# oscka/rag-llm-k8s

Measured on AMD Instinct MI355X. Metric: end-to-end RAG query p50 latency + gen tokens/sec, Llama-3.1-8B top-k=4, higher is better.
Workload: dtype bf16; 1 GPU; model=Llama-3.1-8B-Instruct, embedder=all-MiniLM-L6-v2, index=FlatL2 10000 vectors (HBM-resident; 10000 embedded chunks), retrieve_k=4, context_k=4, global_batch=32, seq_len=5192, parallelism=dp1

## Files before the change

### csrc/kernels/attention.hip

```cpp
#include "common.h"
#include "kv_fp8.h"
#include <type_traits>
using namespace ragk;

namespace {

constexpr int KT = 64;
constexpr int MAX_BT = 2048;
constexpr float RESCALE_LOG2 = 8.f;

__device__ __forceinline__ float max_xor32(float v) {
  const auto r = __builtin_amdgcn_permlane32_swap(__float_as_uint(v), __float_as_uint(v), false, false);
  return fmaxf(__uint_as_float(r[0]), __uint_as_float(r[1]));
}
__device__ __forceinline__ float max_xor16(float v) {
  const auto r = __builtin_amdgcn_permlane16_swap(__float_as_uint(v), __float_as_uint(v), false, false);
  return fmaxf(__uint_as_float(r[0]), __uint_as_float(r[1]));
}

template <int D>
struct Cfg {
  static constexpr int NC = D / 8;
  static constexpr int ROWB = D * 2;
  static constexpr int TILEB = KT * D * 2;
  static constexpr int PIECES = TILEB / 1024;
  static constexpr int RPP = 1024 / ROWB;
  static constexpr int KS = D / 32;
  static constexpr int DT = D / 16;
  static constexpr int GR = D / 16;
  static constexpr int RB = 8 / GR;
};

template <int D>
__device__ __forceinline__ int kswz(int row) {
  constexpr int NC = Cfg<D>::NC;
  return (row / (16 / NC)) & (NC - 1);
}
template <int D>
__device__ __forceinline__ int vswz(int row) {
  return 2 * ((row / Cfg<D>::RB) & (Cfg<D>::GR - 1));
}

__device__ __forceinline__ bf16x4 tr_read(const char* p) {
  return __builtin_amdgcn_ds_read_tr16_b64_v4i16((__attribute__((address_space(3))) bf16x4*)(p));
}

template <int D, bool IS_V, bool NT = false, int NW = 0, typename RowSrc>
__device__ __forceinline__ void stage_kv(char* lds_tile, int wid, int nwaves, int lane, RowSrc row_src) {
  constexpr int NC = Cfg<D>::NC, PIECES = Cfg<D>::PIECES, RPP = Cfg<D>::RPP;
  constexpr int PPW = NW > 0 ? PIECES / NW : PIECES;
#pragma unroll
  for (int i = 0; i < PPW; ++i) {
    const int p = NW > 0 ? wid + NW * i : wid + nwaves * i;
    if (NW == 0 && p >= PIECES) break;
    const int row = p * RPP + lane / NC;
    const int ph = lane % NC;
    const int c = ph ^ (IS_V ? vswz<D>(row) : kswz<D>(row));
    if constexpr (NT)
      __builtin_amdgcn_global_load_lds((const __attribute__((address_space(1))) void*)(row_src(row) + c * 8),
                                       (__attribute__((address_space(3))) void*)(lds_tile + p * 1024), 16, 0, 2);
    else
      glds16(row_src(row) + c * 8, lds_tile + p * 1024);
  }
}

template <int D>
__device__ __forceinline__ bf16x8 load_vt(const char* sV, int dt, int ks, int lane) {
  const int h = lane >> 4, i = lane & 15;
  const int chunk = 2 * dt + ((i >> 1) & 1);
  const int r0 = 32 * ks + 4 * h + (i >> 2);
  const int r1 = r0 + 16;
  const bf16x4 a = tr_read(sV + r0 * Cfg<D>::ROWB + 16 * (chunk ^ vswz<D>(r0)) + 8 * (i & 1));
  const bf16x4 b = tr_read(sV + r1 * Cfg<D>::ROWB + 16 * (chunk ^ vswz<D>(r1)) + 8 * (i & 1));
  return (bf16x8){a[0], a[1], a[2], a[3], b[0], b[1], b[2], b[3]};
}

template <int D>
__device__ __forceinline__ bf16x8 load_k(const char* sK, int t, int s, int lane) {
  const int R = 16 * t + (lane & 15);
  const int c = 4 * s + (lane >> 4);
  return *reinterpret_cast<const bf16x8*>(sK + R * Cfg<D>::ROWB + 16 * (c ^ kswz<D>(R)));
}

__device__ __forceinline__ bf16x8 pack_p(const f32x4& a, const f32x4& b) {
  return (bf16x8){f2bf_s(a[0]), f2bf_s(a[1]), f2bf_s(a[2]), f2bf_s(a[3]),
                  f2bf_s(b[0]), f2bf_s(b[1]), f2bf_s(b[2]), f2bf_s(b[3])};
}

constexpr int F8_D = 128;
constexpr int F8_TILEB = KT * F8_D;

__device__ __forceinline__ int f8_qoff(int s, int fh) { return 64 * (s >> 1) + 16 * fh + 8 * (s & 1); }

template <bool NT>
__device__ __forceinline__ u32x4 f8_ld16(const unsigned char* p) {
  if constexpr (NT) return __builtin_nontemporal_load(reinterpret_cast<const u32x4*>(p));
  else return *reinterpret_cast<const u32x4*>(p);
}

__device__ __forceinline__ void f8_v_to_lds(char* sV, int ci, const u32x4 raw) {
  const int row = ci >> 3, c = ci & 7;
  char* p = sV + row * Cfg<F8_D>::ROWB + 16 * ((2 * c) ^ vswz<F8_D>(row));
  *reinterpret_cast<bf16x8*>(p) = kv8_to_bf16(raw[0], raw[1]);
  *reinterpret_cast<bf16x8*>(p + 16) = kv8_to_bf16(raw[2], raw[3]);
}

__device__ __forceinline__ void f8_load_k(const char* sK, int t, int j, int lane, bf16x8& k0, bf16x8& k1) {
  const u32x4 raw = __builtin_bit_cast(u32x4, load_k<64>(sK, t, j, lane));
  k0 = kv8_to_bf16(raw[0], raw[1]);
  k1 = kv8_to_bf16(raw[2], raw[3]);
}

struct PrefillArgs {
  const bf16_t* q;  int q_stride;
  const bf16_t* k;  const bf16_t* v;
  int kv_stride;
  const int* block_tables; int bt_stride;
  const int* cu_q;
  const int* cu_kv;
  const int* kv_lens;
  const int* tiles;
  bf16_t* out; int out_stride;
  int Hq, Hkv;
  float scale_log2;
  unsigned kv_bytes;
  int n_hg;
  const float* ks; const float* vs;
};

__device__ inline void prefill_block(const PrefillArgs& a, int& tile, int& hg) {
  if (a.n_hg > 0) {
    tile = (int)blockIdx.x / a.n_hg;
    hg = (int)blockIdx.x - tile * a.n_hg;
  } else {
    tile = blockIdx.x;
    hg = blockIdx.y;
  }
}

template <int D, int GB, bool CAUSAL, bool PAGED, int NWV = 4, bool F8 = false>
__global__ __launch_bounds__(NWV * 64, 8 / NWV) void attn_prefill_kernel(PrefillArgs a) {
  static_assert(!F8 || (PAGED && D == F8_D), "fp8 cache: paged, D = 128");
  using C = Cfg<D>;
  constexpr int NTH = NWV * 64;
  constexpr int QT = 32 * (NWV / GB);
// ... 540 lines not shown
      fast(P3{}, t + 2, S1, S0);
      fast(P0{}, t + 3, S0, S1);
    }
    if (t < t_end) {
      fast(P1{}, t, S1, S0);
      ++t;
    }
    if (t < t_end) {
      fast(P2{}, t, S0, S1);
      ++t;
    }
    if (t < t_end) {
      fast(P3{}, t, S1, S0);
      ++t;
    }
    if (t & 1) {
#pragma unroll
      for (int kb = 0; kb < 2; ++kb) S0[kb] = S1[kb];
    }
  }
  if (t + 2 < n_kt) stage(t + 2, true);
  wait_vmcnt0();
  barrier();
  if (t >= 1) pv_simple(t - 1);
  for (; t < n_kt; ++t) {
    const int k0 = t * KT;
    const bool need_mask = (k0 + KT - 1 > ctx0 + pbase) || (k0 + KT > kv_len);
    const float alpha = need_mask ? softmax(std::true_type{}, k0, S0) : softmax(std::false_type{}, k0, S0);
    rescale(alpha);
    pv_simple(t);
    if (t + 1 < n_kt) qk_simple(t + 1, S0);
  }

  const auto lr = __builtin_amdgcn_permlane32_swap(__float_as_uint(l_i), __float_as_uint(l_i), false, false);
  const float l = __uint_as_float(lr[0]) + __uint_as_float(lr[1]);
  const float inv = l > 0.f ? 1.f / l : 0.f;
  __syncthreads();
  char* so = smem + wid_u * 8192;
#pragma unroll
  for (int db = 0; db < 4; ++db)
#pragma unroll
    for (int b = 0; b < 4; ++b) {
      const int e = 4 * b;
      const int d = 32 * db + 8 * b + 4 * h;
      const int c = (d >> 3) ^ (l32 & 15);
      *reinterpret_cast<uint2*>(so + l32 * 256 + 16 * c + 8 * ((d >> 2) & 1)) =
          make_uint2(pk2bf(o[db][e] * inv, o[db][e + 1] * inv), pk2bf(o[db][e + 2] * inv, o[db][e + 3] * inv));
    }
  asm volatile("s_waitcnt lgkmcnt(0)" ::: "memory");
#pragma unroll
  for (int i = 0; i < 8; ++i) {
    const int r = 4 * i + (lane >> 4), c = lane & 15;
    const u32x4 v = *reinterpret_cast<const u32x4*>(so + r * 256 + 16 * (c ^ (r & 15)));
    if (pbase + r < q_len)
      *reinterpret_cast<u32x4*>(a.out + (size_t)(q_off + pbase + r) * a.out_stride + hq * D + 8 * c) = v;
  }
}

struct DecodeArgs {
  const bf16_t* q; int q_stride;
  const bf16_t* kc; const bf16_t* vc;
  const int* block_tables; int bt_stride;
  const int* kv_lens;
  float* part_o;
  float* part_ml;
  bf16_t* out; int out_stride;
  int Hq, Hkv, part_tiles, max_parts;
  float scale_log2;
  const float* qkv_p; long long p_slab; int ldp, S;
  const int* positions; const int* slots;
  const float* cos_t; const float* sin_t;
  const float* ks; const float* vs;
};

__device__ __forceinline__ int decode_part_tiles(int n_kt, const DecodeArgs& a) {
  return max(a.part_tiles, (n_kt + a.max_parts - 1) / a.max_parts);
}

template <int D, int G, int NW = 4, bool KL = false, bool F8 = false>
constexpr int decode_lds_bytes() {
  return F8 ? NW * (Cfg<D>::TILEB + (KL ? F8_TILEB : 0)) + G * D * 2 : NW * Cfg<D>::TILEB * (KL ? 2 : 1) + G * D * 2;
}

template <int D, int G, bool NT = false, int NW = 4, int DG = 0, bool KL = false, bool F8 = false>
__device__ __forceinline__ void attn_decode_block(const DecodeArgs& a, int part, int kvh, int b, char* smem) {
  constexpr int NTH = NW * 64;
  using C = Cfg<D>;
  static_assert(G <= 16, "at most 16 query heads per KV head");
  static_assert(!F8 || (D == F8_D && DG == 0), "fp8 cache: D = 128");
  const int lane = threadIdx.x & 63, wid = threadIdx.x >> 6;
  const int wid_u = __builtin_amdgcn_readfirstlane(wid);
  const int kv_len = a.kv_lens[b];
  const int n_kt = (kv_len + KT - 1) / KT;
  const int pt = decode_part_tiles(n_kt, a);
  const int kt0 = part * pt;
  if (kt0 >= n_kt) return;
  const int kt1 = min(kt0 + pt, n_kt);
  const int nparts = (n_kt + pt - 1) / pt;
  const int fr = lane & 15, fh = lane >> 4;
  const int* bt = a.block_tables + (size_t)b * a.bt_stride;

  bf16x8 qf[C::KS];
  char* sV = smem + wid * C::TILEB;
  char* sK = F8 ? smem + NW * C::TILEB + wid * F8_TILEB : smem + (NW + wid) * C::TILEB;
  const bool pre = !F8 && a.qkv_p != nullptr && kt0 + wid_u < kt1 && kt0 + wid_u != n_kt - 1;
  bf16x8 kf0[4][C::KS];
  if (pre) {
    const size_t base = ((size_t)bt[kt0 + wid_u] * a.Hkv + kvh) * KT * D;
    const bf16_t* kb = a.kc + base;
    const bf16_t* vb = a.vc + base;
    if constexpr (KL) stage_kv<D, false, NT, 1>(sK, 0, 1, lane, [&](int r) { return kb + (size_t)r * D; });
    stage_kv<D, true, NT, 1>(sV, 0, 1, lane, [&](int r) { return vb + (size_t)r * D; });
#pragma unroll
    for (int t = 0; t < 4; ++t)
#pragma unroll
      for (int s = 0; s < C::KS; ++s)
        if constexpr (!KL)
          kf0[t][s] = NT ? __builtin_nontemporal_load(reinterpret_cast<const bf16x8*>(kb + (size_t)(16 * t + fr) * D +
                                                                                     32 * s + 8 * fh))
                         : *reinterpret_cast<const bf16x8*>(kb + (size_t)(16 * t + fr) * D + 32 * s + 8 * fh);
  }
  if (a.qkv_p != nullptr) {
    bf16_t* s_q = reinterpret_cast<bf16_t*>(smem + decode_lds_bytes<D, G, NW, KL, F8>() - G * D * 2);
    constexpr int NV = D / 16;
    const int pos = a.positions[b];
    const float* prow = a.qkv_p + (size_t)b * a.ldp;
    const float* ct = a.cos_t + (size_t)pos * (D / 2);
    const float* st = a.sin_t + (size_t)pos * (D / 2);
    const int tid = threadIdx.x;
    const bool append = kt1 == n_kt;
    constexpr int KV0 = (G * NV + 63) / 64 * 64;
    if (tid < G * NV) {
      const int g = tid / NV, v = tid % NV;
      const float* ph = prow + (size_t)(kvh * G + g) * D + 8 * v;
      float x1[8], x2[8], o1[8], o2[8];
      sum_partials8x2(ph, ph + D / 2, a.S, (size_t)a.p_slab, x1, x2);
      rope8(x1, x2, ct + 8 * v, st + 8 * v, o1, o2);
      *reinterpret_cast<u32x4*>(s_q + g * D + 8 * v) = pack8(o1);
      *reinterpret_cast<u32x4*>(s_q + g * D + D / 2 + 8 * v) = pack8(o2);
    } else if (append && tid >= KV0 && tid < KV0 + 2 * NV) {
      const int isv = tid - KV0 >= NV, v = (tid - KV0) % NV;
      const int slot = a.slots[b];
      const size_t kvo = (((size_t)(slot / KT) * a.Hkv + kvh) * KT + (slot % KT)) * D;
      const float* ph = prow + (size_t)(a.Hq + (isv ? a.Hkv : 0) + kvh) * D + 8 * v;
      float x1[8], x2[8];
      sum_partials8x2(ph, ph + D / 2, a.S, (size_t)a.p_slab, x1, x2);
      bf16_t* dst = (isv ? const_cast<bf16_t*>(a.vc) : const_cast<bf16_t*>(a.kc)) + kvo;
      if constexpr (F8) {
        float r1[8], r2[8];
        if (isv) {
#pragma unroll
          for (int e = 0; e < 8; ++e) { r1[e] = x1[e]; r2[e] = x2[e]; }
        } else {
          rope8(x1, x2, ct + 8 * v, st + 8 * v, r1, r2);
        }
        unsigned char* base8 = reinterpret_cast<unsigned char*>(const_cast<bf16_t*>(isv ? a.vc : a.kc));
        kv8_store_row128(r1, r2, v, base8 + kvo, const_cast<float*>(isv ? a.vs : a.ks) + kvo / D);
      } else if (isv) {
        *reinterpret_cast<u32x4*>(dst + 8 * v) = pack8(x1);
        *reinterpret_cast<u32x4*>(dst + D / 2 + 8 * v) = pack8(x2);
      } else {
        float o1[8], o2[8];
        rope8(x1, x2, ct + 8 * v, st + 8 * v, o1, o2);
        *reinterpret_cast<u32x4*>(dst + 8 * v) = pack8(o1);
        *reinterpret_cast<u32x4*>(dst + D / 2 + 8 * v) = pack8(o2);
      }
    }
    __syncthreads();
#pragma unroll
    for (int s = 0; s < C::KS; ++s)
      qf[s] = fr < G ? *reinterpret_cast<const bf16x8*>(s_q + fr * D + (F8 ? f8_qoff(s, fh) : 32 * s + 8 * fh))
                     : (bf16x8){0, 0, 0, 0, 0, 0, 0, 0};
  } else {
    const int g = fr < G ? fr : 0;
    const bf16_t* qp = a.q + (size_t)b * a.q_stride + (kvh * G + g) * D + 8 * fh;
#pragma unroll
    for (int s = 0; s < C::KS; ++s) {
      const bf16x8 v = *reinterpret_cast<const bf16x8*>(F8 ? qp - 8 * fh + f8_qoff(s, fh) : qp + 32 * s);
      qf[s] = fr < G ? v : (bf16x8){0, 0, 0, 0, 0, 0, 0, 0};
    }
  }
  f32x4 o[C::DT];
#pragma unroll
  for (int dt = 0; dt < C::DT; ++dt) o[dt] = (f32x4){0.f, 0.f, 0.f, 0.f};
  float m_i = -INFINITY, l_i = 0.f;
  unsigned dsink = 0;

  for (int kt = kt0 + wid_u; kt < kt1; kt += NW) {
    bf16x8 kf[4][C::KS];
    u32x4 f8_v[F8 ? 8 : 1];
    f32x4 ksc[4], vsc[4];
    if constexpr (F8) {
      const size_t blk = (size_t)bt[kt] * a.Hkv + kvh;
      const unsigned char* kb = reinterpret_cast<const unsigned char*>(a.kc) + blk * F8_TILEB;
      const unsigned char* vb = reinterpret_cast<const unsigned char*>(a.vc) + blk * F8_TILEB;
      asm volatile("s_waitcnt lgkmcnt(0)" ::: "memory");
      if constexpr (KL)
        stage_kv<64, false, NT, 1>(sK, 0, 1, lane,
                                   [&](int r) { return reinterpret_cast<const bf16_t*>(kb + (size_t)r * F8_D); });
      u32x4 kraw[4][2];
      if constexpr (!KL) {
#pragma unroll
        for (int t = 0; t < 4; ++t)
#pragma unroll
          for (int j = 0; j < 2; ++j) kraw[t][j] = f8_ld16<NT>(kb + (16 * t + fr) * F8_D + 16 * (4 * j + fh));
      }
#pragma unroll
      for (int t = 0; t < 4; ++t) {
        ksc[t] = *reinterpret_cast<const f32x4*>(a.ks + blk * KT + 16 * t + 4 * fh);
        vsc[t] = *reinterpret_cast<const f32x4*>(a.vs + blk * KT + 16 * t + 4 * fh);
      }
#pragma unroll
      for (int i = 0; i < 8; ++i) f8_v[i] = f8_ld16<NT>(vb + 16 * (64 * i + lane));
      if constexpr (KL) {
        __builtin_amdgcn_s_waitcnt((0x7 << 4) | (0xF << 8));
#pragma unroll
        for (int t = 0; t < 4; ++t)
#pragma unroll
          for (int j = 0; j < 2; ++j) f8_load_k(sK, t, j, lane, kf[t][2 * j], kf[t][2 * j + 1]);
      } else {
#pragma unroll
        for (int t = 0; t < 4; ++t)
#pragma unroll
          for (int j = 0; j < 2; ++j) {
            kf[t][2 * j] = kv8_to_bf16(kraw[t][j][0], kraw[t][j][1]);
            kf[t][2 * j + 1] = kv8_to_bf16(kraw[t][j][2], kraw[t][j][3]);
          }
      }
    } else if constexpr (KL) {
      if (!(pre && kt == kt0 + wid_u)) {
        const size_t base = ((size_t)bt[kt] * a.Hkv + kvh) * KT * D;
        const bf16_t* kb = a.kc + base;
        const bf16_t* vb = a.vc + base;
        asm volatile("s_waitcnt lgkmcnt(0)" ::: "memory");
        stage_kv<D, false, NT, 1>(sK, 0, 1, lane, [&](int r) { return kb + (size_t)r * D; });
        stage_kv<D, true, NT, 1>(sV, 0, 1, lane, [&](int r) { return vb + (size_t)r * D; });
      }
      static_assert(Cfg<D>::PIECES < 64, "vmcnt range");
      __builtin_amdgcn_s_waitcnt((Cfg<D>::PIECES & 15) | (((Cfg<D>::PIECES >> 4) & 3) << 14) | (0x7 << 4) | (0xF << 8));
#pragma unroll
      for (int t = 0; t < 4; ++t)
#pragma unroll
        for (int s = 0; s < C::KS; ++s) kf[t][s] = load_k<D>(sK, t, s, lane);
    } else if (pre && kt == kt0 + wid_u) {
#pragma unroll
      for (int t = 0; t < 4; ++t)
#pragma unroll
        for (int s = 0; s < C::KS; ++s) kf[t][s] = kf0[t][s];
    } else if (DG == 2) {
      const size_t base = ((size_t)bt[kt] * a.Hkv + kvh) * KT * D;
      const bf16_t* kb = a.kc + base;
      const bf16_t* vb = a.vc + base;
      asm volatile("s_waitcnt lgkmcnt(0)" ::: "memory");
      stage_kv<D, true, NT, 1>(sV, 0, 1, lane, [&](int r) { return vb + (size_t)r * D; });
      stage_kv<D, false, NT, 1>(sV, 0, 1, lane, [&](int r) { return kb + (size_t)r * D; });
#pragma unroll
      for (int t = 0; t < 4; ++t)
#pragma unroll
        for (int s = 0; s < C::KS; ++s) kf[t][s] = (bf16x8){0, 0, 0, 0, 0, 0, 0, 0};
    } else {
      const size_t base = ((size_t)bt[kt] * a.Hkv + kvh) * KT * D;
      const bf16_t* kb = a.kc + base;
      const bf16_t* vb = a.vc + base;
      asm volatile("s_waitcnt lgkmcnt(0)" ::: "memory");
      stage_kv<D, true, NT, 1>(sV, 0, 1, lane, [&](int r) { return vb + (size_t)r * D; });
#pragma unroll
      for (int t = 0; t < 4; ++t)
#pragma unroll
        for (int s = 0; s < C::KS; ++s)
          kf[t][s] = NT ? __builtin_nontemporal_load(reinterpret_cast<const bf16x8*>(kb + (size_t)(16 * t + fr) * D +
                                                                                    32 * s + 8 * fh))
                        : *reinterpret_cast<const bf16x8*>(kb + (size_t)(16 * t + fr) * D + 32 * s + 8 * fh);
    }
    if constexpr (DG != 0) {
#pragma unroll
      for (int t = 0; t < 4; ++t)
#pragma unroll
        for (int s = 0; s < C::KS; ++s) dsink ^= __builtin_bit_cast(u32x4, kf[t][s])[0];
      wait_vmcnt0();
      dsink ^= *reinterpret_cast<const unsigned*>(sV + 4 * lane);
      continue;
    }
    f32x4 s4[4];
#pragma unroll
    for (int t = 0; t < 4; ++t) {
      s4[t] = (f32x4){0.f, 0.f, 0.f, 0.f};
#pragma unroll
      for (int s = 0; s < C::KS; ++s) s4[t] = __builtin_amdgcn_mfma_f32_16x16x32_bf16(kf[t][s], qf[s], s4[t], 0, 0, 0);
    }
    const int k0 = kt * KT;
    float mx = -INFINITY;
#pragma unroll
    for (int t = 0; t < 4; ++t)
#pragma unroll
      for (int r = 0; r < 4; ++r) {
        const int kj = k0 + 16 * t + 4 * fh + r;
        const float x = kj < kv_len ? (F8 ? s4[t][r] * ksc[t][r] : s4[t][r]) * a.scale_log2 : -INFINITY;
        s4[t][r] = x;
        mx = fmaxf(mx, x);
      }
    mx = fmaxf(mx, __shfl_xor(mx, 16, 64));
    mx = fmaxf(mx, __shfl_xor(mx, 32, 64));
    const float m_new = fmaxf(m_i, mx);
    const float m_use = m_new == -INFINITY ? 0.f : m_new;
    const float alpha = __builtin_amdgcn_exp2f(m_i - m_use);
    float ls = 0.f;
#pragma unroll
    for (int t = 0; t < 4; ++t)
#pragma unroll
      for (int r = 0; r < 4; ++r) {
        const float p = __builtin_amdgcn_exp2f(s4[t][r] - m_use);
        ls += p;
        if constexpr (F8)
          s4[t][r] = k0 + 16 * t + 4 * fh + r < kv_len ? p * vsc[t][r] : 0.f;
        else
          s4[t][r] = p;
      }
    l_i = l_i * alpha + ls;
    m_i = m_new;
#pragma unroll
    for (int dt = 0; dt < C::DT; ++dt) o[dt] *= alpha;
    const bf16x8 pb0 = pack_p(s4[0], s4[1]);
    const bf16x8 pb1 = pack_p(s4[2], s4[3]);
    if constexpr (F8) {
#pragma unroll
      for (int i = 0; i < 8; ++i) f8_v_to_lds(sV, 64 * i + lane, f8_v[i]);
      asm volatile("" ::: "memory");
    } else if constexpr (KL)
      __builtin_amdgcn_s_waitcnt((0x7 << 4) | (0xF << 8));
    else
      wait_vmcnt0();
#pragma unroll
    for (int dt = 0; dt < C::DT; ++dt) {
      o[dt] = __builtin_amdgcn_mfma_f32_16x16x32_bf16(load_vt<D>(sV, dt, 0, lane), pb0, o[dt], 0, 0, 0);
      o[dt] = __builtin_amdgcn_mfma_f32_16x16x32_bf16(load_vt<D>(sV, dt, 1, lane), pb1, o[dt], 0, 0, 0);
    }
  }

  if constexpr (DG != 0) {
    if (dsink == 0x9e3779b9u) a.out[(size_t)b * a.out_stride + lane] = 0;
    return;
  }
  __syncthreads();
  float* sm = reinterpret_cast<float*>(smem);
  float* sl = sm + NW * 16;
  float* so = sl + NW * 64;
  if (fh == 0) sm[wid * 16 + fr] = m_i;
  sl[wid * 64 + lane] = l_i;
#pragma unroll
  for (int dt = 0; dt < C::DT; ++dt)
#pragma unroll
    for (int r = 0; r < 4; ++r) so[(wid * 16 + fr) * D + 16 * dt + 4 * fh + r] = o[dt][r];
  __syncthreads();
  for (int e = threadIdx.x; e < G * D; e += NTH) {
    const int g = e / D, d = e % D;
    float M = -INFINITY;
#pragma unroll
    for (int w = 0; w < NW; ++w) M = fmaxf(M, sm[w * 16 + g]);
    const float Mu = M == -INFINITY ? 0.f : M;
    float L = 0.f, O = 0.f;
#pragma unroll
    for (int w = 0; w < NW; ++w) {
      const float sc = exp2f(sm[w * 16 + g] - Mu);
      L += (sl[w * 64 + g] + sl[w * 64 + g + 16] + sl[w * 64 + g + 32] + sl[w * 64 + g + 48]) * sc;
      O += so[(w * 16 + g) * D + d] * sc;
    }
    const int hq = kvh * G + g;
    if (nparts == 1) {
      a.out[(size_t)b * a.out_stride + hq * D + d] = f2bf(L > 0.f ? O / L : 0.f);
    } else {
      const size_t pi = ((size_t)b * a.Hq + hq) * a.max_parts + part;
      a.part_o[pi * D + d] = O;
      if (d == 0) {
        a.part_ml[pi * 2] = M;
        a.part_ml[pi * 2 + 1] = L;
      }
    }
  }
}

template <int D, int G, bool NT = false, int NW = 4, int DG = 0, bool KL = false, bool F8 = false>
__global__ __launch_bounds__(NW * 64, (NW == 4 && !KL) ? 2 : 1) void attn_decode_kernel(DecodeArgs a) {
  __shared__ __attribute__((aligned(16))) char smem[decode_lds_bytes<D, G, NW, KL, F8>()];
  attn_decode_block<D, G, NT, NW, DG, KL, F8>(a, blockIdx.x, blockIdx.y, blockIdx.z, smem);
}

constexpr int RED_MAXP = 256;
__global__ void attn_decode_reduce_kernel(DecodeArgs a, int D) {
  __shared__ float s_sc[RED_MAXP];
  __shared__ float s_red[8];
  __shared__ float s_M, s_L;
  const int hq = blockIdx.x, b = blockIdx.y, t = threadIdx.x;
  const int nw = (blockDim.x + 63) >> 6, lane = t & 63, wid = t >> 6;
  const int n_kt = (a.kv_lens[b] + KT - 1) / KT;
  const int pt = decode_part_tiles(n_kt, a);
  const int nparts = (n_kt + pt - 1) / pt;
  if (nparts <= 1) return;
  const size_t p0 = ((size_t)b * a.Hq + hq) * a.max_parts;
  float m = -INFINITY;
  for (int p = t; p < nparts; p += blockDim.x) {
    const float mp = a.part_ml[(p0 + p) * 2];
    s_sc[p] = mp;
    m = fmaxf(m, mp);
  }
  m = wave_max(m);
  if (lane == 0) s_red[wid] = m;
  __syncthreads();
  if (t == 0) {
    float M = -INFINITY;
    for (int w = 0; w < nw; ++w) M = fmaxf(M, s_red[w]);
    s_M = M == -INFINITY ? 0.f : M;
  }
  __syncthreads();
  const float Mu = s_M;
  float l = 0.f;
  for (int p = t; p < nparts; p += blockDim.x) {
    const float sc = exp2f(s_sc[p] - Mu);
    s_sc[p] = sc;
    l += a.part_ml[(p0 + p) * 2 + 1] * sc;
  }
  l = wave_sum(l);
  __syncthreads();
  if (lane == 0) s_red[wid] = l;
  __syncthreads();
  if (t == 0) {
    float L = 0.f;
    for (int w = 0; w < nw; ++w) L += s_red[w];
    s_L = L;
  }
  __syncthreads();
  if (t >= D) return;
  const float* po = a.part_o + p0 * D + t;
  float O = 0.f;
  int p = 0;
  for (; p + 8 <= nparts; p += 8) {
    float v[8];
#pragma unroll
    for (int i = 0; i < 8; ++i) v[i] = po[(size_t)(p + i) * D];
#pragma unroll
    for (int i = 0; i < 8; ++i) O += v[i] * s_sc[p + i];
  }
  for (; p < nparts; ++p) O += po[(size_t)p * D] * s_sc[p];
  const float L = s_L;
  a.out[(size_t)b * a.out_stride + hq * D + t] = f2bf(L > 0.f ? O / L : 0.f);
}

template <int D, int GB, bool CAUSAL, bool PAGED, bool F8 = false>
hipError_t launch_prefill(PrefillArgs a, int n_tiles, hipStream_t st) {
  const int G = a.Hq / a.Hkv;
  const int n_hg = a.Hkv * (G / GB);
  a.n_hg = n_hg;
  const dim3 grid(n_tiles * n_hg);
  if constexpr (D == 128 && GB == 4 && CAUSAL && PAGED && !F8) {
    if (a.kv_bytes) {
      hipLaunchKernelGGL(attn_prefill_v3_kernel, grid, dim3(512), 0, st, a);
      return hipGetLastError();
    }
  }
  if constexpr (GB == 4)
    hipLaunchKernelGGL((attn_prefill_kernel<D, GB, CAUSAL, PAGED, 8, F8>), grid, dim3(512), 0, st, a);
  else
    hipLaunchKernelGGL((attn_prefill_kernel<D, GB, CAUSAL, PAGED, 4, F8>), grid, dim3(256), 0, st, a);
  return hipGetLastError();
}

}

RAGK_API int ragk_attn_prefill_qtile(int Hq, int Hkv) {
  const int G = Hq / Hkv;
  const int GB = G % 4 == 0 ? 4 : (G % 2 == 0 ? 2 : 1);
  return 32 * ((GB == 4 ? 8 : 4) / GB);
}

RAGK_API int ragk_attn_prefill(const void* q, int q_stride, const void* k, const void* v, const float* ks,
                               const float* vs, int kv_stride, const int* block_tables, int bt_stride,
                               const int* cu_q, const int* cu_kv, const int* kv_lens, const int* tiles, int n_tiles,
                               void* out, int out_stride, int Hq, int Hkv, int D, int causal, int paged, float scale,
                               hipStream_t st) {
  if (n_tiles <= 0) return 0;
  if (Hq % Hkv || (ks != nullptr) != (vs != nullptr)) return (int)hipErrorInvalidValue;
  if (ks && (D != 128 || !paged || !causal || !k || !v || !block_tables)) return (int)hipErrorInvalidValue;
  const unsigned long long cache_bytes = paged && !ks ? (unsigned long long)kv_stride * Hkv * KT * D * 2 : 0ull;
  PrefillArgs a{(const bf16_t*)q, q_stride, (const bf16_t*)k, (const bf16_t*)v, kv_stride, block_tables, bt_stride,
                cu_q, cu_kv, kv_lens, tiles, (bf16_t*)out, out_stride, Hq, Hkv, scale * 1.4426950408889634f,
                cache_bytes < (1ull << 32) ? (unsigned)cache_bytes : 0u, 0, ks, vs};
  const int G = Hq / Hkv;
  const int GB = G % 4 == 0 ? 4 : (G % 2 == 0 ? 2 : 1);
  if (ks) {
    if (GB == 4) return (int)launch_prefill<128, 4, true, true, true>(a, n_tiles, st);
    if (GB == 2) return (int)launch_prefill<128, 2, true, true, true>(a, n_tiles, st);
    return (int)launch_prefill<128, 1, true, true, true>(a, n_tiles, st);
  }
#define RAGK_PF(DD, GG, CC, PP)                                                          \
  if (D == DD && GB == GG && (bool)causal == CC && (bool)paged == PP)                      \
    return (int)launch_prefill<DD, GG, CC, PP>(a, n_tiles, st);
  RAGK_PF(128, 4, true, true)
  RAGK_PF(128, 1, true, true)
  RAGK_PF(128, 2, true, true)
  RAGK_PF(64, 1, true, true)
  RAGK_PF(64, 4, true, true)
  RAGK_PF(128, 4, true, false)
  RAGK_PF(64, 1, false, false)
  RAGK_PF(32, 1, false, false)
  RAGK_PF(128, 1, false, false)
  RAGK_PF(64, 1, true, false)
#undef RAGK_PF
  return (int)hipErrorInvalidValue;
}

enum : unsigned {
  DEC_NT = 1u << 0,
  DEC_SINGLE = 1u << 1,
  DEC_KL = 1u << 2,
  DEC_DEFER_MERGE = 1u << 3,
  DEC_DIAG_SHIFT = 4,
  DEC_ALL = 0x3fu,
};

static int launch_attn_decode_fp8(DecodeArgs a, int B, int D, int max_parts, unsigned flags, hipStream_t st) {
  const int Hq = a.Hq, Hkv = a.Hkv;
  const int G = Hq / Hkv;
  if (D != 128) return (int)hipErrorInvalidValue;
  dim3 grid(max_parts, Hkv, B);
  if (G == 4 && max_parts == 1 && (flags & DEC_KL) && (flags & DEC_SINGLE)) {
    if (flags & DEC_NT)
      hipLaunchKernelGGL((attn_decode_kernel<128, 4, true, 4, 0, true, true>), grid, dim3(256), 0, st, a);
    else
      hipLaunchKernelGGL((attn_decode_kernel<128, 4, false, 4, 0, true, true>), grid, dim3(256), 0, st, a);
    return (int)hipGetLastError();
  }
#define RAGK_DC8(GG)                                                                               \
  if (G == GG) {                                                                                   \
    if (flags & DEC_NT)                                                                            \
      hipLaunchKernelGGL((attn_decode_kernel<128, GG, true, 4, 0, false, true>), grid, dim3(256), 0, st, a);  \
    else                                                                                           \
      hipLaunchKernelGGL((attn_decode_kernel<128, GG, false, 4, 0, false, true>), grid, dim3(256), 0, st, a); \
    if (max_parts > 1 && !(flags & DEC_DEFER_MERGE))                                               \
      hipLaunchKernelGGL(attn_decode_reduce_kernel, dim3(Hq, B), dim3(128), 0, st, a, 128);        \
    return (int)hipGetLastError();                                                                 \
  }
  RAGK_DC8(4)
  RAGK_DC8(8)
  RAGK_DC8(1)
  RAGK_DC8(2)
#undef RAGK_DC8
  return (int)hipErrorInvalidValue;
}

static int launch_attn_decode(DecodeArgs a, int B, int D, int max_parts, unsigned flags, hipStream_t st) {
  const int Hq = a.Hq, Hkv = a.Hkv;
  const int G = Hq / Hkv;
  const unsigned diag = (flags >> DEC_DIAG_SHIFT) & 3u;
  if (a.ks) return launch_attn_decode_fp8(a, B, D, max_parts, flags, st);
  dim3 grid(max_parts, Hkv, B);
  if (D == 128 && G == 4 && max_parts == 1 && (flags & DEC_SINGLE)) {
    if ((flags & DEC_KL) && !diag)
      hipLaunchKernelGGL((attn_decode_kernel<128, 4, true, 4, 0, true>), grid, dim3(256), 0, st, a);
    else if (diag == 1)
      hipLaunchKernelGGL((attn_decode_kernel<128, 4, true, 8, 1>), grid, dim3(512), 0, st, a);
    else if (diag == 2)
      hipLaunchKernelGGL((attn_decode_kernel<128, 4, true, 8, 2>), grid, dim3(512), 0, st, a);
    else if (flags & DEC_NT)
      hipLaunchKernelGGL((attn_decode_kernel<128, 4, true, 8>), grid, dim3(512), 0, st, a);
    else
      hipLaunchKernelGGL((attn_decode_kernel<128, 4, false, 8>), grid, dim3(512), 0, st, a);
    return (int)hipGetLastError();
  }
#define RAGK_DC(DD, GG)                                                            \
  if (D == DD && G == GG) {                                                          \
    if (flags & DEC_NT)                                                              \
      hipLaunchKernelGGL((attn_decode_kernel<DD, GG, true>), grid, dim3(256), 0, st, a); \
    else                                                                             \
      hipLaunchKernelGGL((attn_decode_kernel<DD, GG, false>), grid, dim3(256), 0, st, a); \
    if (max_parts > 1 && !(flags & DEC_DEFER_MERGE))                                 \
      hipLaunchKernelGGL(attn_decode_reduce_kernel, dim3(Hq, B), dim3(DD), 0, st, a, DD); \
    return (int)hipGetLastError();                                                   \
  }
  RAGK_DC(128, 4)
  RAGK_DC(128, 8)
  RAGK_DC(128, 1)
  RAGK_DC(64, 1)
  RAGK_DC(64, 4)
  RAGK_DC(128, 2)
#undef RAGK_DC
  return (int)hipErrorInvalidValue;
}

RAGK_API int ragk_attn_decode(const void* q, int q_stride, const float* P, int S, int ldp, const int* positions,
                              const int* slots, const float* cos_t, const float* sin_t, void* kc, void* vc,
                              float* ks, float* vs, const int* block_tables, int bt_stride, const int* kv_lens,
                              float* part_o, float* part_ml, void* out, int out_stride, int B, int Hq, int Hkv,
                              int D, int part_tiles, int max_parts, float scale, unsigned flags, hipStream_t st) {
  if (B <= 0) return 0;
  if (Hq % Hkv || part_tiles < 1 || max_parts < 1 || max_parts > RED_MAXP || (q != nullptr) == (P != nullptr) ||
      (ks != nullptr) != (vs != nullptr) ||
      (flags & ~DEC_ALL) || ((flags >> DEC_DIAG_SHIFT) & 3u) == 3u || (ks && D != 128))
    return (int)hipErrorInvalidValue;
  if (P && (S < 1 || D % 64 || ldp < (Hq + 2 * Hkv) * D || !positions || !slots || !cos_t || !sin_t))
    return (int)hipErrorInvalidValue;
  DecodeArgs a{(const bf16_t*)q, q_stride, (const bf16_t*)kc, (const bf16_t*)vc, block_tables, bt_stride, kv_lens,
               part_o, part_ml, (bf16_t*)out, out_stride, Hq, Hkv, part_tiles, max_parts,
               scale * 1.4426950408889634f};
  if (P) {
    a.qkv_p = P, a.p_slab = (long long)B * ldp, a.ldp = ldp, a.S = S;
    a.positions = positions, a.slots = slots, a.cos_t = cos_t, a.sin_t = sin_t;
  }
  a.ks = ks, a.vs = vs;
  return launch_attn_decode(a, B, D, max_parts, flags, st);
}
```

### rag_llm_k8s_amd/ops/native.py

```python
from __future__ import annotations

import math
import os
import threading

import torch

from . import _lib
from ._lib import check, ptr, stream_ptr
from .fp8 import FP8, Fp8KV
from .reference import EPI


def _req(cond, msg):
    if not cond:
        raise ValueError(msg)


def _kv8(k_cache, v_cache, Hkv, D, dev):
    _req(isinstance(k_cache, Fp8KV) and isinstance(v_cache, Fp8KV), "fp8 KV cache: both k and v must be Fp8KV")
    _req(D == 128, "fp8 KV cache needs head_dim 128")
    kd = k_cache.data
    _req(kd.dim() == 4 and kd.shape[1] == Hkv and kd.shape[2] == 64 and kd.shape[3] == D, "fp8 cache [nb,Hkv,64,128]")
    for side, c in (("k", k_cache), ("v", v_cache)):
# ... 975 lines not shown
    ql = np.asarray(q_lens, dtype=np.int64)
    nt = (ql + qt - 1) // qt
    seq = np.repeat(np.arange(len(ql)), nt)
    first = np.repeat(np.cumsum(nt) - nt, nt)
    q0 = (np.arange(int(nt.sum())) - first) * qt
    order = np.argsort(-q0, kind="stable")
    return torch.from_numpy(np.stack([seq[order], q0[order]], 1).astype(np.int32)).reshape(-1, 2)


M_TILE_ROWS = 256


def build_last_rows_lists(q_lens, rows, Hq, Hkv, tiles=None):
    import numpy as np

    qt = prefill_qtile(Hq, Hkv)
    if tiles is None:
        tiles = build_prefill_tiles(q_lens, Hq, Hkv)
    t = tiles.numpy().reshape(-1, 2).astype(np.int64)
    ql = np.asarray(q_lens, dtype=np.int64)
    cu = np.concatenate([[0], np.cumsum(ql)])
    r = np.unique(np.asarray(rows, dtype=np.int64).reshape(-1))
    if r.size and (r[0] < 0 or r[-1] >= cu[-1]):
        raise ValueError("build_last_rows_lists: row outside the packed step")
    lo = cu[t[:, 0]] + t[:, 1]
    hi = np.minimum(lo + qt, cu[t[:, 0] + 1])
    keep = np.searchsorted(r, lo, side="left") < np.searchsorted(r, hi, side="left")
    tiles_last = torch.from_numpy(np.ascontiguousarray(t[keep]).astype(np.int32)).reshape(-1, 2)
    m_tiles = torch.from_numpy(np.unique(r // M_TILE_ROWS).astype(np.int32))
    return tiles_last, m_tiles


def attn_prefill(q, k, v, cu_q, kv_lens, tiles, out, Hq, Hkv, D, causal=True, paged=True, block_tables=None,
                 cu_kv=None, kv_stride=0, scale=None):
    _req(q.dtype == torch.bfloat16 and q.stride(-1) == 1, "q")
    _req(tiles.dtype == torch.int32 and tiles.is_cuda and tiles.is_contiguous(), "tiles int32 on GPU")
    _req(D in (32, 64, 128), "head_dim must be 32/64/128")
    f8 = isinstance(k, Fp8KV) or isinstance(v, Fp8KV)
    if f8:
        _req(paged and causal, "fp8 KV cache: paged causal attention only")
        _kv8(k, v, Hkv, D, q.device)
    if paged:
        _req(len(k.shape) == 4 and k.shape[2] == 64 and k.shape[1] == Hkv and k.shape[3] == D, "paged cache [nb,Hkv,64,D]")
        _req(v.shape == k.shape, "paged k/v caches differ in shape")
        _req(block_tables is not None and block_tables.dtype == torch.int32, "block_tables int32")
        _req(block_tables.stride(0) <= 2048, "prefill block tables wider than 2048 blocks (128k tokens)")
        kv_stride = k.shape[0]
    scale = 1.0 / math.sqrt(D) if scale is None else scale
    kd, vd, ks, vs = (k.data, v.data, k.scale, v.scale) if f8 else (k, v, None, None)
    check(_lib.lib().ragk_attn_prefill(
        q.data_ptr(), q.stride(0), kd.data_ptr(), vd.data_ptr(), ptr(ks), ptr(vs), kv_stride, ptr(block_tables),
        block_tables.stride(0) if block_tables is not None else 0, cu_q.data_ptr(), ptr(cu_kv), kv_lens.data_ptr(),
        tiles.data_ptr(), tiles.shape[0], out.data_ptr(), out.stride(0), Hq, Hkv, D, int(causal), int(paged),
        float(scale), stream_ptr()), "ragk_attn_prefill")
    return out


DECODE_TARGET_BLOCKS = 512
DECODE_MIN_TILES = 4


def _decode_single(batch, Hkv):
    return DECODE_NW8_MIN_PAIRS > 0 and batch * Hkv >= DECODE_NW8_MIN_PAIRS


def decode_partitions(max_kv_len, batch, Hkv, target_blocks=None, min_tiles=None):
    target_blocks = DECODE_TARGET_BLOCKS if target_blocks is None else target_blocks
    min_tiles = DECODE_MIN_TILES if min_tiles is None else min_tiles
    max_kt = max(1, (max_kv_len + 63) // 64)
    if _decode_single(batch, Hkv):
        return min_tiles, 1
    mp = max(1, min(-(-target_blocks // (batch * Hkv)), -(-max_kt // min_tiles)))
    return min_tiles, mp


DECODE_NW8_MIN_PAIRS = 256


DECODE_NT_MIN_BH = 64


DECODE_KL = os.environ.get("RAGK_DECODE_KL", "1") != "0"

DECODE_DIAG = 0

DEC_NT, DEC_SINGLE, DEC_KL, DEC_DEFER_MERGE, DEC_DIAG_SHIFT = 1, 2, 4, 8, 4


def decode_flags(B, Hkv, defer_merge=False):
    return ((DEC_NT if B * Hkv >= DECODE_NT_MIN_BH else 0) | (DEC_SINGLE if _decode_single(B, Hkv) else 0)
            | (DEC_KL if DECODE_KL else 0) | (DEC_DEFER_MERGE if defer_merge else 0)
            | (DECODE_DIAG << DEC_DIAG_SHIFT))


def _launch_attn_decode(q, rope, k_cache, v_cache, block_tables, kv_lens, out, Hq, Hkv, D, part_tiles, max_parts, ws_o,
                        ws_ml, scale, defer_merge=False):
    B = kv_lens.numel()
    dev = out.device
    f8 = isinstance(k_cache, Fp8KV) or isinstance(v_cache, Fp8KV)
    if f8:
        _kv8(k_cache, v_cache, Hkv, D, dev)
    _req(len(k_cache.shape) == 4 and k_cache.shape[1] == Hkv and k_cache.shape[2] == 64 and k_cache.shape[3] == D,
         "paged cache")
    _req(block_tables.dtype == torch.int32 and block_tables.shape[0] >= B, "block_tables")
    _req(kv_lens.dtype == torch.int32, "kv_lens int32")
    _req(Hq // Hkv <= 16, "G <= 16")
    if max_parts > 1:
        if ws_o is None:
            ws_o = torch.empty((B, Hq, max_parts, D), dtype=torch.float32, device=dev)
            ws_ml = torch.empty((B, Hq, max_parts, 2), dtype=torch.float32, device=dev)
        _req(ws_o.numel() >= B * Hq * max_parts * D and ws_ml.numel() >= B * Hq * max_parts * 2, "workspace")
    if defer_merge:
        _req(max_parts > 1 and ws_o is not None, "deferred merge needs a partition workspace")
    scale = 1.0 / math.sqrt(D) if scale is None else scale
    P, positions, slots, cos_t, sin_t = rope or (None,) * 5
    kd, vd = (k_cache.data, v_cache.data) if f8 else (k_cache, v_cache)
    ks, vs = (k_cache.scale, v_cache.scale) if f8 else (None, None)
    check(_lib.lib().ragk_attn_decode(
        ptr(q), q.stride(0) if q is not None else 0, ptr(P), P.shape[0] if rope else 0, P.shape[2] if rope else 0,
        ptr(positions), ptr(slots), ptr(cos_t), ptr(sin_t), kd.data_ptr(), vd.data_ptr(), ptr(ks), ptr(vs),
        block_tables.data_ptr(), block_tables.stride(0), kv_lens.data_ptr(), ptr(ws_o), ptr(ws_ml), out.data_ptr(),
        out.stride(0), B, Hq, Hkv, D, part_tiles, max_parts, float(scale), decode_flags(B, Hkv, defer_merge),
        stream_ptr()), "ragk_attn_decode")
    return out


def attn_decode(q, k_cache, v_cache, block_tables, kv_lens, out, Hq, Hkv, D, part_tiles, max_parts, ws_o=None,
                ws_ml=None, scale=None):
    return _launch_attn_decode(q, None, k_cache, v_cache, block_tables, kv_lens, out, Hq, Hkv, D, part_tiles,
                               max_parts, ws_o, ws_ml, scale)


def attn_decode_rope(P, positions, cos_t, sin_t, slots, k_cache, v_cache, block_tables, kv_lens, out, Hq, Hkv, D,
                     part_tiles, max_parts, ws_o=None, ws_ml=None, scale=None, defer_merge=False):
    _req(P.dtype == torch.float32 and P.is_contiguous() and P.dim() == 3, "partials")
    S, B, ldp = P.shape
    _req(ldp >= (Hq + 2 * Hkv) * D and D % 64 == 0, "qkv width")
    _req(kv_lens.numel() == B, "one partial row per sequence")
    _req(positions.dtype == torch.int32 and positions.numel() == B, "positions")
    _req(slots is not None and slots.dtype == torch.int32 and slots.numel() == B, "slots")
    return _launch_attn_decode(None, (P, positions, slots, cos_t, sin_t), k_cache, v_cache, block_tables, kv_lens, out,
                               Hq, Hkv, D, part_tiles, max_parts, ws_o, ws_ml, scale, defer_merge)


TOPK_CHUNK = 16384


def topk_chunks(V, K, max_cand=512):
    return max(1, min(V // TOPK_CHUNK, max_cand // K, 64))


def topk_candidates(logits, K, vocab_offset=0, max_cand=512, chunks=None, cand_v=None, cand_i=None):
    _req(logits.dtype == torch.float32 and logits.is_cuda and logits.stride(1) == 1, "logits fp32")
    B, V = logits.shape
    _req(1 <= K <= 256, "1 <= K <= 256")
    chunks = topk_chunks(V, K, max_cand) if chunks is None else int(chunks)
    _req(1 <= chunks <= 64, "1 <= chunks <= 64")
    if cand_v is None:
        cand_v = torch.empty((B, chunks * K), dtype=torch.float32, device=logits.device)
        cand_i = torch.empty((B, chunks * K), dtype=torch.int32, device=logits.device)
    _req(cand_v.shape == (B, chunks * K) and cand_i.shape == (B, chunks * K), "candidate buffers [B, chunks*K]")
    check(_lib.lib().ragk_topk_candidates(logits.data_ptr(), logits.stride(0), B, V, K, vocab_offset, chunks,
                                          cand_v.data_ptr(), cand_i.data_ptr(), stream_ptr()), "ragk_topk_candidates")
    return cand_v, cand_i


SAMPLE_LIST_MERGE = True


def sample_candidates(cand_v, cand_i, temps, top_ks, top_ps, seeds, steps, out_tok=None, out_lp=None, list_len=None):
    B, n = cand_v.shape
    _req(n <= 2048, "<= 2048 candidates")
    _req(temps.dtype == torch.float32 and top_ks.dtype == torch.int32 and top_ps.dtype == torch.float32, "param dtypes")
    _req(seeds.dtype == torch.int64 and steps.dtype == torch.int32, "seeds int64 / steps int32")
    out_tok = torch.empty(B, dtype=torch.int32, device=cand_v.device) if out_tok is None else out_tok
    if list_len and SAMPLE_LIST_MERGE:
        _req(n % list_len == 0, "candidate lists")
        check(_lib.lib().ragk_sample_candidates_lists(cand_v.data_ptr(), cand_i.data_ptr(), B, n, int(list_len),
                                                      temps.data_ptr(), top_ks.data_ptr(), top_ps.data_ptr(),
                                                      seeds.data_ptr(), steps.data_ptr(), out_tok.data_ptr(),
                                                      ptr(out_lp), stream_ptr()), "ragk_sample_candidates_lists")
        return out_tok
    check(_lib.lib().ragk_sample_candidates(cand_v.data_ptr(), cand_i.data_ptr(), B, n, temps.data_ptr(),
                                            top_ks.data_ptr(), top_ps.data_ptr(), seeds.data_ptr(), steps.data_ptr(),
                                            out_tok.data_ptr(), ptr(out_lp), stream_ptr()), "ragk_sample_candidates")
    return out_tok


def logits_proc_max_hist():
    return int(_lib.lib().ragk_logits_proc_max_hist())


def _i32_vec(t, n, dev, name):
    _req(t.dtype == torch.int32 and t.is_cuda and t.device == dev and t.dim() == 1 and t.numel() == n
         and t.is_contiguous(), "%s must be a contiguous int32 [%d] tensor on the launch device" % (name, n))


def _hist_buf(hist, dev):
    _req(hist.dtype == torch.int32 and hist.is_cuda and hist.device == dev and hist.dim() == 2
         and hist.is_contiguous() and hist.shape[0] >= 1 and hist.shape[1] >= 1,
         "hist must be a contiguous int32 [rows, max_len] tensor on the launch device")


def hist_write(ids, rows, pos, hist):
    _hist_buf(hist, hist.device)
    T = ids.numel()
# ... 247 lines not shown
```

Before: 1729 generated tokens/s (aggregate over all GPUs).

## Add software-pipelined streaming loop for bf16 KL single-partition decode attention

Adds a STRM variant of the decode attention kernel that issues asynchronous global-to-LDS loads for the next KV tile through inline asm, with explicit vmcnt waits. K and V fragments are read into registers before the next tile's loads are issued into the same LDS buffer. Block-table entries are prefetched 64 at a time into a VGPR and broadcast with readlane. The intent is to overlap HBM loads of tile i+1 with compute on tile i and to cut per-tile global block-table reads. It costs extra registers for the V fragments and adds fragile hand-managed waitcnt and m0 handling.

```diff
diff --git a/csrc/kernels/attention.hip b/csrc/kernels/attention.hip
--- a/csrc/kernels/attention.hip
+++ b/csrc/kernels/attention.hip
@@ -31,6 +31,8 @@
   static constexpr int RB = 8 / GR;
 };
 
+constexpr int vmcnt_imm(int n) { return (n & 15) | (((n >> 4) & 3) << 14) | (0x7 << 4) | (0xF << 8); }
+
 template <int D>
 __device__ __forceinline__ int kswz(int row) {
   constexpr int NC = Cfg<D>::NC;
@@ -61,6 +63,30 @@
                                        (__attribute__((address_space(3))) void*)(lds_tile + p * 1024), 16, 0, 2);
     else
       glds16(row_src(row) + c * 8, lds_tile + p * 1024);
+  }
+}
+
+template <bool NT>
+__device__ __forceinline__ void glds16_asm(const void* gsrc, unsigned lds_dst) {
+  unsigned keep;
+  if constexpr (NT)
+    asm volatile("s_mov_b32 %0, m0\n\ts_mov_b32 m0, %2\n\ts_nop 0\n\tglobal_load_lds_dwordx4 %1, off nt\n\t"
+                 "s_mov_b32 m0, %0"
+                 : "=&s"(keep) : "v"(gsrc), "s"(lds_dst) : "memory");
+  else
+    asm volatile("s_mov_b32 %0, m0\n\ts_mov_b32 m0, %2\n\ts_nop 0\n\tglobal_load_lds_dwordx4 %1, off\n\t"
+                 "s_mov_b32 m0, %0"
+                 : "=&s"(keep) : "v"(gsrc), "s"(lds_dst) : "memory");
+}
+
+template <int D, bool IS_V, bool NT, typename RowSrc>
+__device__ __forceinline__ void stage_kv_asm(unsigned lds_tile, int lane, RowSrc row_src) {
+  constexpr int NC = Cfg<D>::NC, PIECES = Cfg<D>::PIECES, RPP = Cfg<D>::RPP;
+#pragma unroll
+  for (int p = 0; p < PIECES; ++p) {
+    const int row = p * RPP + lane / NC;
+    const int c = (lane % NC) ^ (IS_V ? vswz<D>(row) : kswz<D>(row));
+    glds16_asm<NT>(row_src(row) + c * 8, lds_tile + p * 1024);
   }
 }
 
@@ -767,12 +793,13 @@
   return F8 ? NW * (Cfg<D>::TILEB + (KL ? F8_TILEB : 0)) + G * D * 2 : NW * Cfg<D>::TILEB * (KL ? 2 : 1) + G * D * 2;
 }
 
-template <int D, int G, bool NT = false, int NW = 4, int DG = 0, bool KL = false, bool F8 = false>
+template <int D, int G, bool NT = false, int NW = 4, int DG = 0, bool KL = false, bool F8 = false, bool STRM = false>
 __device__ __forceinline__ void attn_decode_block(const DecodeArgs& a, int part, int kvh, int b, char* smem) {
   constexpr int NTH = NW * 64;
   using C = Cfg<D>;
   static_assert(G <= 16, "at most 16 query heads per KV head");
   static_assert(!F8 || (D == F8_D && DG == 0), "fp8 cache: D = 128");
+  static_assert(!STRM || (KL && !F8 && DG == 0 && C::PIECES < 32), "stream loop: the bf16 KL kernel");
   const int lane = threadIdx.x & 63, wid = threadIdx.x >> 6;
   const int wid_u = __builtin_amdgcn_readfirstlane(wid);
   const int kv_len = a.kv_lens[b];
@@ -789,13 +816,34 @@
   char* sV = smem + wid * C::TILEB;
   char* sK = F8 ? smem + NW * C::TILEB + wid * F8_TILEB : smem + (NW + wid) * C::TILEB;
   const bool pre = !F8 && a.qkv_p != nullptr && kt0 + wid_u < kt1 && kt0 + wid_u != n_kt - 1;
+  const unsigned sK_a = lds_addr(smem) + (NW + wid_u) * C::TILEB, sV_a = lds_addr(smem) + wid_u * C::TILEB;
+  int btv = 0;
+  auto bt_fill = [&](int j0) {
+    const int t = kt0 + wid_u + NW * (j0 + lane);
+    btv = t < kt1 ? bt[t] : 0;
+    asm volatile("" : "+v"(btv));
+  };
+  auto issue_k = [&](int j) {
+    const bf16_t* kb = a.kc + ((size_t)__builtin_amdgcn_readlane(btv, j & 63) * a.Hkv + kvh) * KT * D;
+    stage_kv_asm<D, false, NT>(sK_a, lane, [&](int r) { return kb + (size_t)r * D; });
+  };
+  auto issue_v = [&](int j) {
+    const bf16_t* vb = a.vc + ((size_t)__builtin_amdgcn_readlane(btv, j & 63) * a.Hkv + kvh) * KT * D;
+    stage_kv_asm<D, true, NT>(sV_a, lane, [&](int r) { return vb + (size_t)r * D; });
+  };
+  if constexpr (STRM) bt_fill(0);
   bf16x8 kf0[4][C::KS];
   if (pre) {
     const size_t base = ((size_t)bt[kt0 + wid_u] * a.Hkv + kvh) * KT * D;
     const bf16_t* kb = a.kc + base;
     const bf16_t* vb = a.vc + base;
-    if constexpr (KL) stage_kv<D, false, NT, 1>(sK, 0, 1, lane, [&](int r) { return kb + (size_t)r * D; });
-    stage_kv<D, true, NT, 1>(sV, 0, 1, lane, [&](int r) { return vb + (size_t)r * D; });
+    if constexpr (STRM) {
+      issue_k(0);
+      issue_v(0);
+    } else {
+      if constexpr (KL) stage_kv<D, false, NT, 1>(sK, 0, 1, lane, [&](int r) { return kb + (size_t)r * D; });
+      stage_kv<D, true, NT, 1>(sV, 0, 1, lane, [&](int r) { return vb + (size_t)r * D; });
+    }
 #pragma unroll
     for (int t = 0; t < 4; ++t)
 #pragma unroll
@@ -864,6 +912,7 @@
       const bf16x8 v = *reinterpret_cast<const bf16x8*>(F8 ? qp - 8 * fh + f8_qoff(s, fh) : qp + 32 * s);
       qf[s] = fr < G ? v : (bf16x8){0, 0, 0, 0, 0, 0, 0, 0};
     }
+    if constexpr (STRM) __builtin_amdgcn_s_waitcnt((0x7 << 4) | (0xF << 8));
   }
   f32x4 o[C::DT];
 #pragma unroll
@@ -871,11 +920,29 @@
   float m_i = -INFINITY, l_i = 0.f;
   unsigned dsink = 0;
 
-  for (int kt = kt0 + wid_u; kt < kt1; kt += NW) {
+  int it = 0;
+  for (int kt = kt0 + wid_u; kt < kt1; kt += NW, ++it) {
     bf16x8 kf[4][C::KS];
+    bf16x8 vf[STRM ? C::DT : 1][2];
     u32x4 f8_v[F8 ? 8 : 1];
     f32x4 ksc[4], vsc[4];
-    if constexpr (F8) {
+    const bool more = kt + NW < kt1;
+    if constexpr (STRM) {
+      if (it == 0 && !pre) {
+        issue_k(0);
+        issue_v(0);
+      }
+      if (more && ((it + 1) & 63) == 0) bt_fill(it + 1);
+      __builtin_amdgcn_s_waitcnt(vmcnt_imm(C::PIECES));
+      asm volatile("" ::: "memory");
+#pragma unroll
+      for (int t = 0; t < 4; ++t)
+#pragma unroll
+        for (int s = 0; s < C::KS; ++s) kf[t][s] = load_k<D>(sK, t, s, lane);
+      asm volatile("s_waitcnt lgkmcnt(0)" ::: "memory");
+      if (more) issue_k(it + 1);
+      __builtin_amdgcn_sched_barrier(0);
+    } else if constexpr (F8) {
       const size_t blk = (size_t)bt[kt] * a.Hkv + kvh;
       const unsigned char* kb = reinterpret_cast<const unsigned char*>(a.kc) + blk * F8_TILEB;
       const unsigned char* vb = reinterpret_cast<const unsigned char*>(a.vc) + blk * F8_TILEB;
@@ -973,6 +1040,21 @@
 #pragma unroll
       for (int s = 0; s < C::KS; ++s) s4[t] = __builtin_amdgcn_mfma_f32_16x16x32_bf16(kf[t][s], qf[s], s4[t], 0, 0, 0);
     }
+    if constexpr (STRM) {
+      if (more)
+        __builtin_amdgcn_s_waitcnt(vmcnt_imm(C::PIECES));
+      else
+        __builtin_amdgcn_s_waitcnt(vmcnt_imm(0));
+      asm volatile("" ::: "memory");
+#pragma unroll
+      for (int dt = 0; dt < C::DT; ++dt) {
+        vf[dt][0] = load_vt<D>(sV, dt, 0, lane);
+        vf[dt][1] = load_vt<D>(sV, dt, 1, lane);
+      }
+      asm volatile("s_waitcnt lgkmcnt(0)" ::: "memory");
+      if (more) issue_v(it + 1);
+      __builtin_amdgcn_sched_barrier(0);
+    }
     const int k0 = kt * KT;
     float mx = -INFINITY;
 #pragma unroll
@@ -1011,14 +1093,20 @@
 #pragma unroll
       for (int i = 0; i < 8; ++i) f8_v_to_lds(sV, 64 * i + lane, f8_v[i]);
       asm volatile("" ::: "memory");
+    } else if constexpr (STRM) {
     } else if constexpr (KL)
       __builtin_amdgcn_s_waitcnt((0x7 << 4) | (0xF << 8));
     else
       wait_vmcnt0();
 #pragma unroll
     for (int dt = 0; dt < C::DT; ++dt) {
-      o[dt] = __builtin_amdgcn_mfma_f32_16x16x32_bf16(load_vt<D>(sV, dt, 0, lane), pb0, o[dt], 0, 0, 0);
-      o[dt] = __builtin_amdgcn_mfma_f32_16x16x32_bf16(load_vt<D>(sV, dt, 1, lane), pb1, o[dt], 0, 0, 0);
+      if constexpr (STRM) {
+        o[dt] = __builtin_amdgcn_mfma_f32_16x16x32_bf16(vf[dt][0], pb0, o[dt], 0, 0, 0);
+        o[dt] = __builtin_amdgcn_mfma_f32_16x16x32_bf16(vf[dt][1], pb1, o[dt], 0, 0, 0);
+      } else {
+        o[dt] = __builtin_amdgcn_mfma_f32_16x16x32_bf16(load_vt<D>(sV, dt, 0, lane), pb0, o[dt], 0, 0, 0);
+        o[dt] = __builtin_amdgcn_mfma_f32_16x16x32_bf16(load_vt<D>(sV, dt, 1, lane), pb1, o[dt], 0, 0, 0);
+      }
     }
   }
 
@@ -1064,10 +1152,10 @@
   }
 }
 
-template <int D, int G, bool NT = false, int NW = 4, int DG = 0, bool KL = false, bool F8 = false>
+template <int D, int G, bool NT = false, int NW = 4, int DG = 0, bool KL = false, bool F8 = false, bool STRM = false>
 __global__ __launch_bounds__(NW * 64, (NW == 4 && !KL) ? 2 : 1) void attn_decode_kernel(DecodeArgs a) {
   __shared__ __attribute__((aligned(16))) char smem[decode_lds_bytes<D, G, NW, KL, F8>()];
-  attn_decode_block<D, G, NT, NW, DG, KL, F8>(a, blockIdx.x, blockIdx.y, blockIdx.z, smem);
+  attn_decode_block<D, G, NT, NW, DG, KL, F8, STRM>(a, blockIdx.x, blockIdx.y, blockIdx.z, smem);
 }
 
 constexpr int RED_MAXP = 256;
@@ -1199,7 +1287,8 @@
   DEC_KL = 1u << 2,
   DEC_DEFER_MERGE = 1u << 3,
   DEC_DIAG_SHIFT = 4,
-  DEC_ALL = 0x3fu,
+  DEC_KL_STREAM = 1u << 6,
+  DEC_ALL = 0x7fu,
 };
 
 static int launch_attn_decode_fp8(DecodeArgs a, int B, int D, int max_parts, unsigned flags, hipStream_t st) {
@@ -1239,7 +1328,9 @@
   if (a.ks) return launch_attn_decode_fp8(a, B, D, max_parts, flags, st);
   dim3 grid(max_parts, Hkv, B);
   if (D == 128 && G == 4 && max_parts == 1 && (flags & DEC_SINGLE)) {
-    if ((flags & DEC_KL) && !diag)
+    if ((flags & DEC_KL) && !diag && (flags & DEC_KL_STREAM))
+      hipLaunchKernelGGL((attn_decode_kernel<128, 4, true, 4, 0, true, false, true>), grid, dim3(256), 0, st, a);
+    else if ((flags & DEC_KL) && !diag)
       hipLaunchKernelGGL((attn_decode_kernel<128, 4, true, 4, 0, true>), grid, dim3(256), 0, st, a);
     else if (diag == 1)
       hipLaunchKernelGGL((attn_decode_kernel<128, 4, true, 8, 1>), grid, dim3(512), 0, st, a);
diff --git a/rag_llm_k8s_amd/ops/native.py b/rag_llm_k8s_amd/ops/native.py
--- a/rag_llm_k8s_amd/ops/native.py
+++ b/rag_llm_k8s_amd/ops/native.py
@@ -1081,15 +1081,24 @@
 
 DECODE_KL = os.environ.get("RAGK_DECODE_KL", "1") != "0"
 
+DECODE_KL_STREAM = os.environ.get("RAGK_DECODE_KL_STREAM", "1") != "0"
+
 DECODE_DIAG = 0
 
 DEC_NT, DEC_SINGLE, DEC_KL, DEC_DEFER_MERGE, DEC_DIAG_SHIFT = 1, 2, 4, 8, 4
-
-
-def decode_flags(B, Hkv, defer_merge=False):
-    return ((DEC_NT if B * Hkv >= DECODE_NT_MIN_BH else 0) | (DEC_SINGLE if _decode_single(B, Hkv) else 0)
+DEC_KL_STREAM = 64
+
+
+def decode_flags(B, Hkv, defer_merge=False, kl_route=False):
+    single = _decode_single(B, Hkv)
+    stream = kl_route and single and DECODE_KL and DECODE_KL_STREAM and not DECODE_DIAG
+    return ((DEC_NT if B * Hkv >= DECODE_NT_MIN_BH else 0) | (DEC_SINGLE if single else 0)
             | (DEC_KL if DECODE_KL else 0) | (DEC_DEFER_MERGE if defer_merge else 0)
-            | (DECODE_DIAG << DEC_DIAG_SHIFT))
+            | (DECODE_DIAG << DEC_DIAG_SHIFT) | (DEC_KL_STREAM if stream else 0))
+
+
+def decode_kl_route(f8, Hq, Hkv, D, max_parts):
+    return not f8 and D == 128 and Hq == 4 * Hkv and max_parts == 1
 
 
 def _launch_attn_decode(q, rope, k_cache, v_cache, block_tables, kv_lens, out, Hq, Hkv, D, part_tiles, max_parts, ws_o,
@@ -1119,8 +1128,8 @@
         ptr(q), q.stride(0) if q is not None else 0, ptr(P), P.shape[0] if rope else 0, P.shape[2] if rope else 0,
         ptr(positions), ptr(slots), ptr(cos_t), ptr(sin_t), kd.data_ptr(), vd.data_ptr(), ptr(ks), ptr(vs),
         block_tables.data_ptr(), block_tables.stride(0), kv_lens.data_ptr(), ptr(ws_o), ptr(ws_ml), out.data_ptr(),
-        out.stride(0), B, Hq, Hkv, D, part_tiles, max_parts, float(scale), decode_flags(B, Hkv, defer_merge),
-        stream_ptr()), "ragk_attn_decode")
+        out.stride(0), B, Hq, Hkv, D, part_tiles, max_parts, float(scale),
+        decode_flags(B, Hkv, defer_merge, decode_kl_route(f8, Hq, Hkv, D, max_parts)), stream_ptr()), "ragk_attn_decode")
     return out
 
 
```

After: 1735 generated tokens/s (aggregate over all GPUs) (median of 6 runs). Within noise of the previous version (+0.3%).
